# William-wAng618/roboticAttack

Measured on AMD Instinct MI355X. Metric: attack-steps/sec (bs=64, 3x50x50 patch, OpenVLA-7B), higher is better.
Workload: dtype bf16; 1 GPU; UADA_wrapper_ddp inner step: bs=64/rank (global 64), patch 3,50,50, geometry=True, maskidx=[0]; OpenVLA-7B shape, random init; u8 frames resident in HBM; global_batch=64, parallelism=dp1, regions=weak, visible_gpus=1, labelled_rows_per_rank=128, tunableop_entries_loaded_min_over_ranks=173

## Files before the change

include/vaa_model_ops.h:

```cpp
#ifndef VAA_MODEL_OPS_H_
#define VAA_MODEL_OPS_H_
#include <stdint.h>
#ifdef __cplusplus
extern "C" {
#endif
int vaa_model_rope(const uint16_t* x, long sb, long st, long sh, const float* cos_t, const float* sin_t, int B, int T, int H, int hd,
                   float sin_sign, uint16_t* out, void* stream);
int vaa_model_swiglu_fwd(const uint16_t* gate, const uint16_t* up, uint16_t* y, long n, void* stream);
int vaa_model_swiglu_bwd(const uint16_t* dy, const uint16_t* gate, const uint16_t* up, uint16_t* dgate, uint16_t* dup, long n, void* stream);
int vaa_model_scale_add(const uint16_t* x, const uint16_t* a, const uint16_t* ls, uint16_t* out, long rows, int D, void* stream);
int vaa_model_rmsnorm_fwd(const uint16_t* x, const uint16_t* w, uint16_t* h, float* rstd, long rows, int D, float eps, void* stream);
int vaa_model_rmsnorm_bwd(const uint16_t* gh, const uint16_t* gpass, const uint16_t* x, const uint16_t* w, const float* rstd, uint16_t* gx,
                          long rows, int D, void* stream);
int vaa_model_layernorm_fwd(const uint16_t* x, const uint16_t* w, const uint16_t* b, uint16_t* h, float* stats, long rows, int D, float eps,
                            void* stream);
int vaa_model_layernorm_bwd(const uint16_t* gh, const uint16_t* gpass, const uint16_t* x, const uint16_t* w, const float* stats, uint16_t* gx,
                            long rows, int D, void* stream);
int vaa_model_attention_fwd(const uint16_t* q, const int64_t* q_str, const uint16_t* k, const int64_t* k_str, const uint16_t* v,
                            const int64_t* v_str, uint16_t* o, const int64_t* o_str, float* lse, const int32_t* cu_seqlens, int B, int H,
                            int T, int hd, int causal, float scale, void* stream);
int vaa_model_attention_bwd(const uint16_t* q, const int64_t* q_str, const uint16_t* k, const int64_t* k_str, const uint16_t* v,
                            const int64_t* v_str, const uint16_t* o, const int64_t* o_str, const uint16_t* dout, const int64_t* do_str,
                            const float* lse, float* dsum, uint16_t* dq, const int64_t* dq_str, uint16_t* dk, const int64_t* dk_str,
                            uint16_t* dv, const int64_t* dv_str, const float* rope_cos, const float* rope_sin, const int32_t* cu_seqlens, int B,
                            int H, int T, int hd, int causal, float scale, void* stream);
int vaa_model_attention_decode(const uint16_t* q, const int64_t* q_str, const uint16_t* k_new, const int64_t* k_str, const uint16_t* v_new,
                               const int64_t* v_str, uint16_t* kcache, const int64_t* kc_str, uint16_t* vcache, const int64_t* vc_str,
                               const int32_t* pos, const float* cos_t, const float* sin_t, uint16_t* o, const int64_t* o_str, int B, int H,
                               int Tmax, int hd, float scale, void* stream);
int vaa_model_q4_dequant(const uint8_t* codes, const float* absmax, const float* table, int N, int K, uint16_t* out_bf16, void* stream);
int vaa_model_q4_gemv(const uint16_t* x, int M, const uint8_t* codes, const float* absmax, const float* table, int N, int K,
                      const uint16_t* res, uint16_t* y, void* stream);
int vaa_model_q8_act_quant(const uint16_t* x, int M, int K, float threshold, int8_t* xq, float* ascale, int32_t* outliers, void* stream);
int vaa_model_q8_matmul(const int8_t* xq, const float* ascale, const int32_t* outliers, const uint16_t* x, int M, const int8_t* q,
                        const float* wscale, int N, int K, const uint16_t* res, uint16_t* y, int form, void* stream);
#ifdef __cplusplus
}
#endif
#endif
```

roboticattack_amd/_lib.py:

```python
from __future__ import annotations

import ctypes as C
import os

_HERE = os.path.dirname(os.path.abspath(__file__))
LIB_PATH = os.environ.get("VAA_LIB_PATH") or os.path.join(_HERE, "libvaa_hip.so")

VAA_OK = 0
MASK_LT_M20, MASK_NE_M100 = 0, 1
LOSS_UADA, LOSS_UADA_DDP, LOSS_UPA, LOSS_CE = 0, 1, 2, 3
DTYPE_F32, DTYPE_BF16 = 0, 1
LAYOUT_FULL, LAYOUT_ROWS = 0, 1
GRAD_FULL, GRAD_SLICE = 0, 1
SEG_UPA_MAX_GROUPS = 32
OPT_ADAMW_HF, OPT_PGD_SIGN = 0, 1
FRAME_RESIZE_MAX_TAPS = 57

MODEL_OP_EXPORTS = ("vaa_model_rope", "vaa_model_swiglu_fwd", "vaa_model_swiglu_bwd", "vaa_model_rmsnorm_fwd", "vaa_model_rmsnorm_bwd",
                    "vaa_model_attention_fwd", "vaa_model_attention_bwd", "vaa_model_layernorm_fwd", "vaa_model_layernorm_bwd", "vaa_model_scale_add",
                    "vaa_model_attention_decode", "vaa_model_q8_act_quant", "vaa_model_q8_matmul", "vaa_model_q4_dequant", "vaa_model_q4_gemv")

EXPORTS = (
    "vaa_last_error",
    "vaa_version",
    "vaa_device_check",
    "vaa_patch_apply_fwd",
    "vaa_patch_grad_ws_bytes",
    "vaa_patch_grad_gather",
    "vaa_loss_ws_bytes",
    "vaa_loss_fwd_bwd",
    "vaa_loss_fwd_bwd_ex",
    "vaa_patch_update",
    "vaa_patch_apply_eval",
    "vaa_eval_preprocess",
    "vaa_frame_resize_taps_bytes",
    "vaa_frame_resize",
    "vaa_crop_resize_fwd",
    "vaa_crop_resize_bwd",
    "vaa_scene_jitter_ws_bytes",
    "vaa_scene_jitter_fwd",
    "vaa_scene_jitter_bwd",
    "vaa_defocus_blur_fwd",
    "vaa_defocus_blur_bwd",
    "vaa_jpeg_roundtrip_ws_bytes",
    "vaa_jpeg_roundtrip",
    "vaa_patch_embed_grad_ws_bytes",
    "vaa_patch_embed_grad_gather",
    "vaa_patch_embed_packed_elems",
    "vaa_patch_embed_pack_weights",
    "vaa_patch_embed_grad_multi_ws_bytes",
    "vaa_patch_embed_grad_gather_multi",
    "vaa_patch_resize_fwd",
    "vaa_patch_resize_ws_bytes",
    "vaa_patch_resize_bwd",
    "vaa_patch_jitter_fwd",
    "vaa_patch_jitter_ws_bytes",
    "vaa_patch_jitter_bwd",
    "vaa_patch_reg_parts",
    "vaa_patch_reg",
    "vaa_patch_apply_fwd_multi",
    "vaa_patch_grad_gather_multi",
    "vaa_loss_rowmap_bytes",
    "vaa_loss_rowmap_build",
    "vaa_loss_rows_ws_bytes",
    "vaa_loss_rows_fwd_bwd",
    "vaa_patch_apply_fwd_tiles",
    "vaa_patch_grad_partials",
    "vaa_patch_embed_grad_gather_multi_tiles",
    "vaa_patch_embed_grad_gather_tiles",
    "vaa_loss_rows_stats",
    "vaa_head_loss_ws_bytes",
    "vaa_head_loss_rows_applies",
    "vaa_head_loss_rows_stats",
    "vaa_head_loss_rows_finish",
    "vaa_head_slice_applies",
    "vaa_head_slice_ws_bytes",
    "vaa_head_slice_pack",
    "vaa_head_slice_fwd_bwd",
    "vaa_step_epilogue",
    "vaa_step_epilogue_update",
    "vaa_loss_rowmap_seg_bytes",
    "vaa_loss_rowmap_build_seg",
    "vaa_step_epilogue_seg",
    "vaa_step_epilogue_seg_update",
    "vaa_patch_update_seg",
    "vaa_loss_rows_fwd_bwd_seg",
    "vaa_step_epilogue_seg_tail",
    "vaa_step_epilogue_seg_tail_update",
    "vaa_loss_rows_fwd_bwd_seg_upa",
    "vaa_async_error",
    "vaa_prof_start",
    "vaa_prof_stop",
    "vaa_prof_get",
)


class VaaError(RuntimeError):
    pass


_lib = None


# ... 137 lines not shown
    L.vaa_patch_embed_grad_gather_tiles.argtypes = [vp, i32, vp, i32, vp, vp, vp, vp, vp, vp, vp, i32, i32, i32, i32, i32, C.POINTER(f32), i32, vp, vp, sz, vp]
    L.vaa_loss_rows_stats.restype = i32
    L.vaa_loss_rows_stats.argtypes = [vp, i32, vp, i32, i32, i32, i32, i32, C.POINTER(f32), vp, i32, vp, sz, vp]
    L.vaa_head_loss_ws_bytes.restype = sz
    L.vaa_head_loss_ws_bytes.argtypes = [i32, i32]
    L.vaa_head_loss_rows_applies.restype = i32
    L.vaa_head_loss_rows_applies.argtypes = [i32, i32, i32]
    L.vaa_head_loss_rows_stats.restype = i32
    L.vaa_head_loss_rows_stats.argtypes = [vp, vp, i32, vp, i32, i32, i32, i32, i32, C.POINTER(f32), vp, vp, sz, vp, sz, vp, vp]
    L.vaa_head_loss_rows_finish.restype = i32
    L.vaa_head_loss_rows_finish.argtypes = [vp, i32, i32, i32, i32, i32, C.POINTER(f32), vp, sz, vp, sz, vp, vp, vp, vp, vp]
    L.vaa_head_slice_applies.restype = i32
    L.vaa_head_slice_applies.argtypes = [i32, i32, i32]
    L.vaa_head_slice_ws_bytes.restype = sz
    L.vaa_head_slice_ws_bytes.argtypes = [i32]
    L.vaa_head_slice_pack.restype = i32
    L.vaa_head_slice_pack.argtypes = [vp, i32, i32, vp, vp]
    L.vaa_head_slice_fwd_bwd.restype = i32
    L.vaa_head_slice_fwd_bwd.argtypes = [vp, vp, vp, i32, vp, i32, i32, i32, i32, i32, C.POINTER(f32), vp, vp, vp, sz, vp, vp, vp, vp, sz, vp]
    L.vaa_step_epilogue.restype = i32
    L.vaa_step_epilogue.argtypes = [vp, i32, i32, vp, i32, i32, i32, i32, i32, C.POINTER(f32), vp, sz, vp, vp, vp, vp, vp]
    L.vaa_step_epilogue_update.restype = i32
    L.vaa_step_epilogue_update.argtypes = [vp, i32, i32, vp, i32, i32, i32, i32, i32, C.POINTER(f32), vp, sz, vp, vp, vp, vp, vp, vp, vp, i32, f32, f32, f32, f32,
                                           i32, vp, vp]
    L.vaa_loss_rowmap_seg_bytes.restype = sz
    L.vaa_loss_rowmap_seg_bytes.argtypes = [i32, i32, i32]
    L.vaa_loss_rowmap_build_seg.restype = i32
    L.vaa_loss_rowmap_build_seg.argtypes = [vp, i32, i32, i32, vp, sz, vp]
    L.vaa_step_epilogue_seg.restype = i32
    L.vaa_step_epilogue_seg.argtypes = [vp, i32, i32, i32, vp, i32, i32, i32, i32, i32, C.POINTER(f32), vp, sz, vp, vp, vp, vp, vp]
    L.vaa_step_epilogue_seg_update.restype = i32
    L.vaa_step_epilogue_seg_update.argtypes = [vp, i32, i32, i32, vp, i32, i32, i32, i32, i32, C.POINTER(f32), vp, sz, vp, vp, vp, vp, vp, vp, vp, i32, f32,
                                               f32, f32, f32, i32, vp, vp]
    L.vaa_patch_update_seg.restype = i32
    L.vaa_patch_update_seg.argtypes = [vp, vp, vp, vp, i32, i32, i32, f32, f32, f32, f32, i32, f32, f32, vp, vp]
    L.vaa_loss_rows_fwd_bwd_seg.restype = i32
    L.vaa_loss_rows_fwd_bwd_seg.argtypes = [vp, i32, vp, i32, i32, i32, i32, i32, i32, C.POINTER(f32), vp, vp, vp, vp, i32, vp, sz, vp]
    L.vaa_step_epilogue_seg_tail.restype = i32
    L.vaa_step_epilogue_seg_tail.argtypes = [vp, i32, i32, i32, vp, vp, vp]
    L.vaa_step_epilogue_seg_tail_update.restype = i32
    L.vaa_step_epilogue_seg_tail_update.argtypes = [vp, i32, i32, i32, vp, vp, vp, vp, vp, i32, f32, f32, f32, f32, i32, vp, vp]
    L.vaa_loss_rows_fwd_bwd_seg_upa.restype = i32
    L.vaa_loss_rows_fwd_bwd_seg_upa.argtypes = [vp, i32, vp, i32, i32, i32, i32, i32, C.POINTER(f32), vp, vp, vp, vp, vp, sz, vp]
    L.vaa_async_error.restype = i32
    L.vaa_async_error.argtypes = []
    L.vaa_prof_start.restype = i32
    L.vaa_prof_start.argtypes = [i32]
    L.vaa_prof_stop.restype = i32
    L.vaa_prof_stop.argtypes = []
    L.vaa_prof_get.restype = i32
    L.vaa_prof_get.argtypes = [i32, C.POINTER(C.c_char_p), C.POINTER(f32)]
    lng = C.c_long
    L.vaa_model_rope.restype = i32
    L.vaa_model_rope.argtypes = [vp, lng, lng, lng, vp, vp, i32, i32, i32, i32, f32, vp, vp]
    L.vaa_model_swiglu_fwd.restype = i32
    L.vaa_model_swiglu_fwd.argtypes = [vp, vp, vp, lng, vp]
    L.vaa_model_swiglu_bwd.restype = i32
    L.vaa_model_swiglu_bwd.argtypes = [vp, vp, vp, vp, vp, lng, vp]
    L.vaa_model_scale_add.restype = i32
    L.vaa_model_scale_add.argtypes = [vp, vp, vp, vp, lng, i32, vp]
    L.vaa_model_rmsnorm_fwd.restype = i32
    L.vaa_model_rmsnorm_fwd.argtypes = [vp, vp, vp, vp, lng, i32, f32, vp]
    L.vaa_model_rmsnorm_bwd.restype = i32
    L.vaa_model_rmsnorm_bwd.argtypes = [vp, vp, vp, vp, vp, vp, lng, i32, vp]
    L.vaa_model_layernorm_fwd.restype = i32
    L.vaa_model_layernorm_fwd.argtypes = [vp, vp, vp, vp, vp, lng, i32, f32, vp]
    L.vaa_model_layernorm_bwd.restype = i32
    L.vaa_model_layernorm_bwd.argtypes = [vp, vp, vp, vp, vp, vp, lng, i32, vp]
    i64p = C.POINTER(C.c_int64)
    L.vaa_model_attention_fwd.restype = i32
    L.vaa_model_attention_fwd.argtypes = [vp, i64p, vp, i64p, vp, i64p, vp, i64p, vp, vp, i32, i32, i32, i32, i32, f32, vp]
    L.vaa_model_attention_bwd.restype = i32
    L.vaa_model_attention_bwd.argtypes = [vp, i64p, vp, i64p, vp, i64p, vp, i64p, vp, i64p, vp, vp, vp, i64p, vp, i64p, vp, i64p, vp, vp, vp, i32, i32, i32, i32, i32, f32, vp]
    L.vaa_model_attention_decode.restype = i32
    L.vaa_model_attention_decode.argtypes = [vp, i64p, vp, i64p, vp, i64p, vp, i64p, vp, i64p, vp, vp, vp, vp, i64p, i32, i32, i32, i32, f32, vp]
    L.vaa_model_q4_dequant.restype = i32
    L.vaa_model_q4_dequant.argtypes = [vp, vp, C.POINTER(f32), i32, i32, vp, vp]
    L.vaa_model_q4_gemv.restype = i32
    L.vaa_model_q4_gemv.argtypes = [vp, i32, vp, vp, C.POINTER(f32), i32, i32, vp, vp, vp]
    L.vaa_model_q8_act_quant.restype = i32
    L.vaa_model_q8_act_quant.argtypes = [vp, i32, i32, f32, vp, vp, vp, vp]
    L.vaa_model_q8_matmul.restype = i32
    L.vaa_model_q8_matmul.argtypes = [vp, vp, vp, vp, i32, vp, vp, i32, i32, vp, vp, i32, vp]
    _lib = L
    return L


def check(rc: int, what: str) -> None:
    if rc != VAA_OK:
        msg = lib().vaa_last_error().decode("utf-8", "replace")
        raise VaaError(f"{what} failed with code {rc}: {msg}")


def f32x(vals):
    return (C.c_float * len(vals))(*[float(v) for v in vals])
```

roboticattack_amd/model_ops.py:

```python
from __future__ import annotations

import os

import torch

from . import _lib


def enabled(x: torch.Tensor) -> bool:
    return x.is_cuda and x.dtype == torch.bfloat16 and not os.environ.get("VAA_NO_FUSED_MODEL_OPS")


def attention_kernel_enabled(ops_on: bool, hd: int) -> bool:
    return bool(ops_on) and not os.environ.get("VAA_NO_FUSED_ATTENTION") and hd % 8 == 0 and hd <= 128


def attention_enabled(x_bthd: torch.Tensor) -> bool:
    return (attention_kernel_enabled(enabled(x_bthd), x_bthd.shape[-1])
            and all(s % 8 == 0 for s in x_bthd.stride()[:-1]) and x_bthd.stride(-1) == 1)


def _stream():
    return torch.cuda.current_stream().cuda_stream

# ... 55 lines not shown
    @staticmethod
    def forward(ctx, x, a, ls):
        ctx.save_for_backward(ls)
        return _scale_add(x.contiguous(), a.contiguous(), ls.contiguous())

    @staticmethod
    def backward(ctx, g):
        (ls,) = ctx.saved_tensors
        g = g.contiguous()
        da = _scale_add(None, g, ls.contiguous()) if ctx.needs_input_grad[1] else None
        return (g if ctx.needs_input_grad[0] else None), da, None


def scale_add(x: torch.Tensor, a: torch.Tensor, ls: torch.Tensor) -> torch.Tensor:
    if (enabled(x) and a.dtype == x.dtype and ls.dtype == x.dtype and x.shape == a.shape and ls.dim() == 1 and ls.shape[0] == x.shape[-1]
            and x.shape[-1] % 8 == 0 and a.device == x.device and ls.device == x.device and not ls.requires_grad
            and os.environ.get("VAA_MODEL_SCALE_ADD", "1") != "0"):
        return ScaleAddFn.apply(x, a, ls)
    return torch.addcmul(x, a, ls)


class ResidualRMSNormFn(torch.autograd.Function):

    @staticmethod
    def forward(ctx, x, weight, eps):
        x = x.contiguous()
        D = x.shape[-1]
        rows = x.numel() // D
        h = torch.empty_like(x)
        rstd = torch.empty(rows, dtype=torch.float32, device=x.device)
        _lib.check(_lib.lib().vaa_model_rmsnorm_fwd(x.data_ptr(), weight.data_ptr(), h.data_ptr(), rstd.data_ptr(), rows, D, float(eps), _stream()),
                   "vaa_model_rmsnorm_fwd")
        ctx.save_for_backward(x, weight, rstd)
        return x, h

    @staticmethod
    def backward(ctx, g_pass, g_h):
        x, weight, rstd = ctx.saved_tensors
        D = x.shape[-1]
        rows = x.numel() // D
        if g_h is None:
            return g_pass, None, None
        g_h = g_h.contiguous()
        gp = g_pass.contiguous() if g_pass is not None else None
        gx = torch.empty_like(x)
        _lib.check(_lib.lib().vaa_model_rmsnorm_bwd(g_h.data_ptr(), gp.data_ptr() if gp is not None else None, x.data_ptr(), weight.data_ptr(),
                                                    rstd.data_ptr(), gx.data_ptr(), rows, D, _stream()), "vaa_model_rmsnorm_bwd")
        return gx, None, None


class ResidualLayerNormFn(torch.autograd.Function):

    @staticmethod
    def forward(ctx, x, weight, bias, eps):
        x = x.contiguous()
        D = x.shape[-1]
        rows = x.numel() // D
        h = torch.empty_like(x)
        stats = torch.empty((rows, 2), dtype=torch.float32, device=x.device)
        _lib.check(_lib.lib().vaa_model_layernorm_fwd(x.data_ptr(), weight.data_ptr(), bias.data_ptr(), h.data_ptr(), stats.data_ptr(), rows, D,
                                                      float(eps), _stream()), "vaa_model_layernorm_fwd")
        ctx.save_for_backward(x, weight, stats)
        return x, h

    @staticmethod
    def backward(ctx, g_pass, g_h):
        x, weight, stats = ctx.saved_tensors
        D = x.shape[-1]
        rows = x.numel() // D
        if g_h is None:
            return g_pass, None, None, None
        g_h = g_h.contiguous()
        gp = g_pass.contiguous() if g_pass is not None else None
        gx = torch.empty_like(x)
        _lib.check(_lib.lib().vaa_model_layernorm_bwd(g_h.data_ptr(), gp.data_ptr() if gp is not None else None, x.data_ptr(), weight.data_ptr(),
                                                      stats.data_ptr(), gx.data_ptr(), rows, D, _stream()), "vaa_model_layernorm_bwd")
        return gx, None, None, None


def tn_dgrad_enabled() -> bool:
    return not os.environ.get("VAA_NO_TN_DGRAD")


class FrozenLinearsFn(torch.autograd.Function):

    @staticmethod
    def forward(ctx, x, res, *ws):
        x2 = x.reshape(-1, x.shape[-1])
        W, Wt = ws[0::2], ws[1::2]
        ctx.wt = Wt
        ctx.xshape = x.shape
        ctx.has_res = res is not None
        if res is not None:
            return (torch.addmm(res.reshape(-1, W[0].shape[0]), x2, W[0].t()).view(*x.shape[:-1], W[0].shape[0]),)
        return tuple(torch.nn.functional.linear(x2, w).view(*x.shape[:-1], w.shape[0]) for w in W)

    @staticmethod
    def backward(ctx, *dys):
        dx = None
        for dy, wt in zip(dys, ctx.wt):
            if dy is None:
                continue
            d2 = dy.reshape(-1, dy.shape[-1])
            if dx is None:
                dx = torch.nn.functional.linear(d2, wt)
            else:
                dx.addmm_(d2, wt.t())
        dx = dx.view(ctx.xshape) if dx is not None else None
        dres = dys[0] if ctx.has_res else None
        return (dx, dres) + (None,) * (2 * len(ctx.wt))


def _str3(x: torch.Tensor):
    import ctypes

    if x.stride(3) != 1:
        raise ValueError("attention operands need a contiguous head dimension")
    return (ctypes.c_int64 * 3)(x.stride(0), x.stride(1), x.stride(2))


def attention_fwd(q: torch.Tensor, k: torch.Tensor, v: torch.Tensor, causal: bool, scale: float | None = None, cu_seqlens=None, max_len: int = 0):
    Bq, T, H, hd = q.shape
    scale = float(hd) ** -0.5 if scale is None else float(scale)
    o = torch.empty((Bq, T, H, hd), dtype=torch.bfloat16, device=q.device)
    B, Tm = (int(cu_seqlens.numel()) - 1, int(max_len)) if cu_seqlens is not None else (Bq, T)
    lse = torch.empty((B, H, Tm), dtype=torch.float32, device=q.device)
    rc = _lib.lib().vaa_model_attention_fwd(q.data_ptr(), _str3(q), k.data_ptr(), _str3(k), v.data_ptr(), _str3(v), o.data_ptr(), _str3(o),
                                            lse.data_ptr(), cu_seqlens.data_ptr() if cu_seqlens is not None else None, B, H, Tm, hd,
                                            int(bool(causal)), scale, _stream())
    _lib.check(rc, "vaa_model_attention_fwd")
    return o, lse


def attention_bwd(q, k, v, o, lse, dout, causal: bool, scale: float, packed_grad: bool = False, rope=None, cu_seqlens=None, max_len: int = 0):
    Bq, T, H, hd = q.shape
    B, Tm = (int(cu_seqlens.numel()) - 1, int(max_len)) if cu_seqlens is not None else (Bq, T)
    if dout.stride(3) != 1:
        dout = dout.contiguous()
    if packed_grad:
        buf = torch.empty((Bq, T, 3, H, hd), dtype=torch.bfloat16, device=q.device)
        dq, dk, dv = buf[:, :, 0], buf[:, :, 1], buf[:, :, 2]
    else:
        buf = None
        dq, dk, dv = (torch.empty((Bq, T, H, hd), dtype=torch.bfloat16, device=q.device) for _ in range(3))
    dsum = torch.empty((B, H, Tm), dtype=torch.float32, device=q.device)
    rc = _lib.lib().vaa_model_attention_bwd(q.data_ptr(), _str3(q), k.data_ptr(), _str3(k), v.data_ptr(), _str3(v), o.data_ptr(), _str3(o),
                                            dout.data_ptr(), _str3(dout), lse.data_ptr(), dsum.data_ptr(), dq.data_ptr(), _str3(dq),
                                            dk.data_ptr(), _str3(dk), dv.data_ptr(), _str3(dv), rope[0].data_ptr() if rope else None,
                                            rope[1].data_ptr() if rope else None, cu_seqlens.data_ptr() if cu_seqlens is not None else None,
                                            B, H, Tm, hd, int(bool(causal)), float(scale), _stream())
    _lib.check(rc, "vaa_model_attention_bwd")
    return buf if packed_grad else (dq, dk, dv)


def rope_in_attention(hd: int) -> bool:
    return hd in (64, 128)


def _attention_forward(ctx, q, k, v, rope, causal, scale, cu_seqlens, max_len, packed_src):
    scale = float(q.shape[-1]) ** -0.5 if scale is None else float(scale)
    if rope is not None:
        q, k = _rope_launch(q, *rope, 1.0), _rope_launch(k, *rope, 1.0)
    o, lse = attention_fwd(q, k, v, causal, scale, cu_seqlens, max_len)
    operands = (q, k, v) if packed_src is None else (q, k, packed_src) if rope is not None else (packed_src,)
    ctx.save_for_backward(o, lse, *operands, *(rope or ()), *([cu_seqlens] if cu_seqlens is not None else []))
    ctx.attn = (bool(causal), scale, int(max_len), packed_src is not None, rope is not None, cu_seqlens is not None)
    return o


def _attention_backward(ctx, dout):
    causal, scale, max_len, packed, roped, has_cu = ctx.attn
    o, lse, *rest = ctx.saved_tensors
    cu = rest.pop() if has_cu else None
    rope = (rest.pop(-2), rest.pop()) if roped else None
    if packed:
        src = rest.pop()
        rest += [src[:, :, z] for z in range(len(rest), 3)]
    g = attention_bwd(*rest, o, lse, dout, causal, scale, packed_grad=packed, rope=rope, cu_seqlens=cu, max_len=max_len)
    return (*((g,) if packed else g), *(None,) * (2 + (4 if roped else 0)))


class AttentionFn(torch.autograd.Function):

    @staticmethod
    def forward(ctx, q, k, v, causal, scale):
        return _attention_forward(ctx, q, k, v, None, causal, scale, None, 0, None)

    backward = staticmethod(_attention_backward)


class RopeAttentionFn(torch.autograd.Function):

    @staticmethod
# ... 67 lines not shown
```

roboticattack_amd/openvla_model.py:

```python
from __future__ import annotations

import os
import types
from dataclasses import dataclass
from typing import NamedTuple

import torch
import torch.nn as nn
import torch.nn.functional as F

from . import model_ops
from .constants import IGNORE_INDEX, MODEL_VOCAB, N_IMG_TOKENS, PAD_ID


@dataclass
class VitCfg:
    dim: int
    depth: int
    heads: int
    mlp: int
    n_prefix: int
    cls_pos: bool
    layerscale: bool

# ... 84 lines not shown
        self.fc1 = nn.Linear(c.dim, c.mlp)
        self.fc2 = nn.Linear(c.mlp, c.dim)
        self.ls1 = nn.Parameter(torch.ones(c.dim)) if c.layerscale else None
        self.ls2 = nn.Parameter(torch.ones(c.dim)) if c.layerscale else None

    def forward(self, x):
        B, T, D = x.shape
        fused_ln = _fused(model_ops.enabled(x), D)
        x, h = _norm(self.norm1, x, fused_ln)
        qkv = self.qkv(h).view(B, T, 3, self.heads, D // self.heads)
        if model_ops.attention_enabled(qkv):
            a = model_ops.PackedAttentionFn.apply(qkv, False, None).reshape(B, T, D)
        else:
            qkv = qkv.permute(2, 0, 3, 1, 4)
            a = F.scaled_dot_product_attention(qkv[0], qkv[1], qkv[2]).transpose(1, 2).reshape(B, T, D)
        a = self.proj(a)
        x = model_ops.scale_add(x, a, self.ls1) if self.ls1 is not None else x + a
        x, h = _norm(self.norm2, x, fused_ln)
        h = self.fc2(F.gelu(self.fc1(h)))
        return model_ops.scale_add(x, h, self.ls2) if self.ls2 is not None else x + h


class Vit(nn.Module):

    def __init__(self, c: VitCfg):
        super().__init__()
        self.c = c
        self.patch_embed = nn.Conv2d(3, c.dim, kernel_size=14, stride=14)
        self.pos_embed = nn.Parameter(torch.zeros(1, N_IMG_TOKENS + (1 if c.cls_pos else 0), c.dim))
        self.prefix = nn.Parameter(torch.zeros(1, c.n_prefix, c.dim)) if c.n_prefix else None
        self.blocks = nn.ModuleList([VitBlock(c) for _ in range(c.depth - 1)])

    def embed_params(self):
        from . import ops
        w = self.patch_embed.weight
        if not (w.is_cuda and w.dtype == torch.bfloat16 and self.c.dim % 64 == 0):
            return w.detach().reshape(self.c.dim, 588), self.patch_embed.bias.detach(), None
        hit = getattr(self, "_embed_wp", None)
        if hit is None or hit[0] != w._version or hit[1] is not w:
            hit = (w._version, w, ops.pack_embed_weights(w.detach().reshape(self.c.dim, 588).t().contiguous()))
            self._embed_wp = hit
        return w.detach().reshape(self.c.dim, 588), self.patch_embed.bias.detach(), hit[2]

    def forward(self, img, embedded=None):
        if embedded is not None:
            x = embedded
        else:
            B0 = img.shape[0]
            tiles = img.reshape(B0, 3, 16, 14, 16, 14).permute(0, 2, 4, 1, 3, 5).reshape(B0, 256, 588)
            x = F.linear(tiles, self.patch_embed.weight.reshape(self.c.dim, 588), self.patch_embed.bias)
        if self.prefix is not None and self.c.cls_pos:
            B = x.shape[0]
            cls = self.prefix[:, :1].expand(B, -1, -1)
            reg = self.prefix[:, 1:].expand(B, -1, -1)
            x = torch.cat([cls, x], dim=1) + self.pos_embed
            x = torch.cat([x[:, :1], reg, x[:, 1:]], dim=1)
        elif self.prefix is not None:
            x = torch.cat([self.prefix.expand(x.shape[0], -1, -1), x + self.pos_embed], dim=1)
        else:
            x = x + self.pos_embed
        for blk in self.blocks:
            x = blk(x)
        return x[:, self.c.n_prefix :]


class RMSNorm(nn.Module):
    def __init__(self, dim, eps):
        super().__init__()
        self.weight = nn.Parameter(torch.ones(dim))
        self.eps = eps

    def forward(self, x):
        return F.rms_norm(x, (x.shape[-1],), self.weight, self.eps)


def _rope(q, k, cos, sin):
    def rot(x):
        x1, x2 = x[..., : x.shape[-1] // 2], x[..., x.shape[-1] // 2 :]
        return torch.cat((-x2, x1), dim=-1)

    return q * cos + rot(q) * sin, k * cos + rot(k) * sin


class Bf16Projections:

    def __init__(self, layer):
        self.layer = layer

    def qkv(self, h2, fused, gemv):
        L = self.layer
        if fused:
            return F.linear(h2, L._wcat(("q_proj", "k_proj", "v_proj"))[0])
        return torch.stack([L.q_proj(h2), L.k_proj(h2), L.v_proj(h2)], dim=1).view(h2.shape[0], -1)

    def o(self, a2, res, gemv):
        return torch.addmm(res, a2, self.layer.o_proj.weight.t())

    def gate_up(self, h2, fused, gemv):
        return self.layer.gate_proj(h2), self.layer.up_proj(h2)

    def down(self, y2, res, fused_mlp, gemv):
        if fused_mlp:
            return torch.addmm(res, y2, self.layer.down_proj.weight.t())
        return res + self.layer.down_proj(y2)


class LlamaLayer(nn.Module):
    quant_type = None

    def __init__(self, c: OpenVLACfg):
        super().__init__()
        d = c.llm_dim
        self.heads = c.llm_heads
        self.input_layernorm = RMSNorm(d, c.rms_eps)
        self.q_proj = nn.Linear(d, d, bias=False)
        self.k_proj = nn.Linear(d, d, bias=False)
        self.v_proj = nn.Linear(d, d, bias=False)
        self.o_proj = nn.Linear(d, d, bias=False)
        self.post_attention_layernorm = RMSNorm(d, c.rms_eps)
        self.gate_proj = nn.Linear(d, c.llm_mlp, bias=False)
        self.up_proj = nn.Linear(d, c.llm_mlp, bias=False)
        self.down_proj = nn.Linear(c.llm_mlp, d, bias=False)
        self._wt_cache = {}
        self.projections = Bf16Projections(self)

    def _wt(self, name):
        w = getattr(self, name).weight
        hit = self._wt_cache.get(name)
        if hit is None or hit[0] != w._version or hit[1] is not w:
            hit = (w._version, w, w.detach().t().contiguous())
            self._wt_cache[name] = hit
        return hit[2]

    def _wcat(self, names):
        ws = [getattr(self, n).weight for n in names]
        key = "+".join(names)
        ver = tuple(w._version for w in ws)
        hit = self._wt_cache.get(key)
        if hit is None or hit[0] != ver or any(a is not b for a, b in zip(hit[1], ws)):
            w = torch.cat([w.detach() for w in ws], 0).contiguous()
            hit = (ver, ws, w, w.t().contiguous())
            self._wt_cache[key] = hit
        return hit[2], hit[3]

    def _lin(self, x, names, res=None):
        ws = [w for n in names for w in (getattr(self, n).weight, self._wt(n))]
        return model_ops.FrozenLinearsFn.apply(x, res, *ws)

    def _qkv(self, h, r):
        B, T, _ = h.shape
        if r.qkv_cat:
            (qkv,) = model_ops.FrozenLinearsFn.apply(h, None, *self._wcat(("q_proj", "k_proj", "v_proj")))
            return qkv.view(B, T, 3, self.heads, -1)
        qkv = self._lin(h, ("q_proj", "k_proj", "v_proj")) if r.tn else (self.q_proj(h), self.k_proj(h), self.v_proj(h))
        return tuple(t.view(B, T, self.heads, -1) for t in qkv)

    def _attention(self, qkv, r, cos, sin, rope_tab):
        if r.attention == "rope_packed":
            return model_ops.RopePackedAttentionFn.apply(qkv, *rope_tab, True, None, r.cu, r.max_len)
        q, k, v = qkv if isinstance(qkv, tuple) else (qkv[:, :, z] for z in range(3))
        if r.attention == "rope":
            return model_ops.RopeAttentionFn.apply(q, k, v, *rope_tab, True, None, r.cu, r.max_len)
        if r.attention != "stock_sdpa":
            q, k = model_ops.RopeFn.apply(q, *rope_tab), model_ops.RopeFn.apply(k, *rope_tab)
        if r.attention == "rope_fn_attention":
            return model_ops.AttentionFn.apply(q, k, v, True, None)
        q, k, v = q.transpose(1, 2), k.transpose(1, 2), v.transpose(1, 2)
        if r.attention == "stock_sdpa":
            q, k = _rope(q, k, cos, sin)
        return F.scaled_dot_product_attention(q, k, v, is_causal=True).transpose(1, 2)

    def _proj_res(self, name, a, x, r):
        if r.tn:
            return self._lin(a, (name,), res=x)[0]
        return torch.addmm(x.reshape(-1, x.shape[-1]), a.reshape(-1, a.shape[-1]), getattr(self, name).weight.t()).view(x.shape)

    def _mlp(self, x, h, r):
        if not (r.fused and (h.shape[0] * h.shape[1] * self.gate_proj.out_features) % 8 == 0):
            return x + self.down_proj(F.silu(self.gate_proj(h)) * self.up_proj(h))
        g, u = self._lin(h, ("gate_proj", "up_proj")) if r.tn else (self.gate_proj(h), self.up_proj(h))
        return self._proj_res("down_proj", model_ops.SwiGLUFn.apply(g, u), x, r)

    def forward(self, x, cos, sin, rope_tab=None, rows=None, pack=None, route=None):
        if self.quant_type:
            from . import quant

            quant.refuse_training("LlamaLayer.forward", self.quant_type)
        B, T, D = x.shape
        r = route if route is not None else _route(rows=B * T, pack=pack, **_facts(x, self.heads, rope_tab))
        x, h = _norm(self.input_layernorm, x, r.fused)
        a = self._attention(self._qkv(h, r), r, cos, sin, rope_tab).reshape(B, T, D)
        if rows is not None:
            a, x = (t.reshape(-1, D).index_select(0, rows)[None] for t in (a, x))
        x = self._proj_res("o_proj", a, x, r)
        x, h = _norm(self.post_attention_layernorm, x, r.fused)
        x = self._mlp(x, h, r)
        return x[0] if rows is not None else x

    def _infer_fused(self, x) -> bool:
        return _fused(model_ops.enabled(x), x.shape[-1], x.shape[-1] // self.heads)

    def _infer_norm_qkv(self, x, fused, gemv):
        B, T, D = x.shape
        h = _norm(self.input_layernorm, x, fused)[1].reshape(-1, D)
        return self.projections.qkv(h, fused, gemv).view(B, T, 3, self.heads, D // self.heads)

    def _infer_o_mlp(self, x, a, fused, gemv):
        B, T, D = x.shape
        proj = self.projections
        x2 = proj.o(a.reshape(-1, D), x.reshape(-1, D), gemv)
        h = _norm(self.post_attention_layernorm, x2.view(B, T, D), fused)[1].reshape(-1, D)
        g, u = proj.gate_up(h, fused, gemv)
        fused_mlp = fused and (B * T * g.shape[1]) % 8 == 0
        y = model_ops.SwiGLUFn.apply(g, u) if fused_mlp else F.silu(g) * u
        return proj.down(y, x2, fused_mlp, gemv).view(B, T, D)

    @torch.no_grad()
    def prefill(self, x, rope_tab, cache):
        B, T, D = x.shape
        fused = self._infer_fused(x)
        qkv = self._infer_norm_qkv(x, fused, gemv=False)
        cos, sin = rope_tab[0][:T], rope_tab[1][:T]
        if fused:
            q, k = model_ops.RopeFn.apply(qkv[:, :, 0], cos, sin), model_ops.RopeFn.apply(qkv[:, :, 1], cos, sin)
        else:
            c, s = (torch.cat([t, t], -1).to(x.dtype)[None, :, None, :] for t in (cos, sin))
            q, k = _rope(qkv[:, :, 0], qkv[:, :, 1], c, s)
        v = qkv[:, :, 2]
        if fused and model_ops.attention_enabled(q):
            a = model_ops.attention_fwd(q, k, v, True)[0]
        else:
            a = F.scaled_dot_product_attention(q.transpose(1, 2), k.transpose(1, 2), v.transpose(1, 2), is_causal=True).transpose(1, 2)
        cache[0][:, :T] = k
        cache[1][:, :T] = v
        return self._infer_o_mlp(x, a.reshape(B, T, D), fused, gemv=False)

    @torch.no_grad()
    def decode_step(self, x, pos, rope_tab, cache):
        B, _, D = x.shape
        fused = self._infer_fused(x)
        qkv = self._infer_norm_qkv(x, fused, gemv=True)[:, 0]
        a = model_ops.attention_decode(qkv[:, 0], qkv[:, 1], qkv[:, 2], cache[0], cache[1], pos, rope_tab[0], rope_tab[1])
        return self._infer_o_mlp(x, a.reshape(B, 1, D), fused, gemv=True)


class SeqPack:

    def __init__(self, attention_mask: torch.Tensor):
        B, L = attention_mask.shape
        self.T_pad = N_IMG_TOKENS + L
        lens = (attention_mask.sum(1).to(torch.int64) + N_IMG_TOKENS).tolist()
        dev = attention_mask.device
        cu = [0]
        for n in lens:
            cu.append(cu[-1] + int(n))
        self.total = cu[-1]
        fill = (-cu[-1]) % 256
        if fill:
# ... 289 lines not shown
```

Before: 2.217 attack-steps/s.

## Route residual linear projections through native hipBLASLt GEMM with TunableOp selections

Adds a native hipBLASLt/rocBLAS GEMM entry point with per-thread cached plans, a registered per-stream workspace, and algorithm selection read from the PyTorch TunableOp CSV. The residual-add projections (o_proj, down_proj) now call it, with C=residual and beta=1, in place of torch.addmm, and a new autograd function covers the untied frozen-weight path. The aim is to skip PyTorch's addmm dispatch and copy overhead and to reuse tuned solutions directly. It adds per-call ctypes overhead and a new code path that may pick different kernels. Weight cache keys now also include the data pointer and shape.

```diff
diff --git a/include/vaa_model_ops.h b/include/vaa_model_ops.h
--- a/include/vaa_model_ops.h
+++ b/include/vaa_model_ops.h
@@ -1,5 +1,6 @@
 #ifndef VAA_MODEL_OPS_H_
 #define VAA_MODEL_OPS_H_
+#include <stddef.h>
 #include <stdint.h>
 #ifdef __cplusplus
 extern "C" {
@@ -34,6 +35,10 @@
 int vaa_model_q8_act_quant(const uint16_t* x, int M, int K, float threshold, int8_t* xq, float* ascale, int32_t* outliers, void* stream);
 int vaa_model_q8_matmul(const int8_t* xq, const float* ascale, const int32_t* outliers, const uint16_t* x, int M, const int8_t* q,
                         const float* wscale, int N, int K, const uint16_t* res, uint16_t* y, int form, void* stream);
+int vaa_model_gemm(const uint16_t* A, long lda, const uint16_t* W, long ldw, const uint16_t* bias, const uint16_t* C, long ldc, uint16_t* D, long ldd,
+                   long M, long N, long K, void* stream);
+int vaa_model_gemm_workspace(void* ws, size_t ws_bytes, void* stream);
+int vaa_model_gemm_tuning_file(const char* path, int device);
 #ifdef __cplusplus
 }
 #endif
diff --git a/roboticattack_amd/_lib.py b/roboticattack_amd/_lib.py
--- a/roboticattack_amd/_lib.py
+++ b/roboticattack_amd/_lib.py
@@ -18,7 +18,8 @@
 
 MODEL_OP_EXPORTS = ("vaa_model_rope", "vaa_model_swiglu_fwd", "vaa_model_swiglu_bwd", "vaa_model_rmsnorm_fwd", "vaa_model_rmsnorm_bwd",
                     "vaa_model_attention_fwd", "vaa_model_attention_bwd", "vaa_model_layernorm_fwd", "vaa_model_layernorm_bwd", "vaa_model_scale_add",
-                    "vaa_model_attention_decode", "vaa_model_q8_act_quant", "vaa_model_q8_matmul", "vaa_model_q4_dequant", "vaa_model_q4_gemv")
+                    "vaa_model_attention_decode", "vaa_model_gemm", "vaa_model_gemm_workspace", "vaa_model_gemm_tuning_file",
+                    "vaa_model_q8_act_quant", "vaa_model_q8_matmul", "vaa_model_q4_dequant", "vaa_model_q4_gemv")
 
 EXPORTS = (
     "vaa_last_error",
@@ -322,6 +323,12 @@
     L.vaa_model_q8_act_quant.argtypes = [vp, i32, i32, f32, vp, vp, vp, vp]
     L.vaa_model_q8_matmul.restype = i32
     L.vaa_model_q8_matmul.argtypes = [vp, vp, vp, vp, i32, vp, vp, i32, i32, vp, vp, i32, vp]
+    L.vaa_model_gemm.restype = i32
+    L.vaa_model_gemm.argtypes = [vp, lng, vp, lng, vp, vp, lng, vp, lng, lng, lng, lng, vp]
+    L.vaa_model_gemm_workspace.restype = i32
+    L.vaa_model_gemm_workspace.argtypes = [vp, sz, vp]
+    L.vaa_model_gemm_tuning_file.restype = i32
+    L.vaa_model_gemm_tuning_file.argtypes = [C.c_char_p, i32]
     _lib = L
     return L
 
diff --git a/roboticattack_amd/csrc/vaa_gemm.hip b/roboticattack_amd/csrc/vaa_gemm.hip
--- /dev/null
+++ b/roboticattack_amd/csrc/vaa_gemm.hip
@@ -0,0 +1,352 @@
+#include <hipblaslt/hipblaslt-ext.hpp>
+#include <hipblaslt/hipblaslt.h>
+#include <rocblas/rocblas.h>
+
+#include <mutex>
+#include <vector>
+
+#include "../../include/vaa_model_ops.h"
+#include "vaa_common.h"
+#include "vaa_gemm_csv.h"
+
+namespace {
+
+using vaa::set_error;
+namespace csv = vaa::gemm_csv;
+
+constexpr int kMaxDevices = 64;
+
+struct WsEntry {
+    int dev;
+    void* stream;
+    void* ptr;
+    size_t bytes;
+};
+std::mutex g_mu;
+csv::Table* g_table[kMaxDevices] = {};
+unsigned g_table_gen = 0;
+std::vector<WsEntry> g_ws;
+
+bool workspace_of(int dev, void* stream, void** ptr, size_t* bytes) {
+    std::lock_guard<std::mutex> lk(g_mu);
+    for (const WsEntry& e : g_ws)
+        if (e.dev == dev && e.stream == stream) {
+            *ptr = e.ptr;
+            *bytes = e.bytes;
+            return true;
+        }
+    *ptr = nullptr;
+    *bytes = 0;
+    return false;
+}
+
+struct Key {
+    int dev;
+    long M, N, K, lda, ldw, ldc, ldd;
+    bool bias, has_c;
+    bool operator==(const Key& o) const {
+        return dev == o.dev && M == o.M && N == o.N && K == o.K && lda == o.lda && ldw == o.ldw && ldc == o.ldc && ldd == o.ldd && bias == o.bias &&
+               has_c == o.has_c;
+    }
+};
+
+struct Plan {
+    Key key;
+    int backend;
+    hipblasLtMatmulDesc_t desc;
+    hipblasLtMatrixLayout_t la, lb, lc, ld;
+    hipblasLtMatmulAlgo_t algo;
+    size_t ws_need;
+    int solution;
+    bool rb_checked;
+    const void* bias_set;
+};
+
+struct ThreadState {
+    hipblasLtHandle_t lt[kMaxDevices];
+    rocblas_handle rb[kMaxDevices];
+    std::vector<Plan>* plans;
+    unsigned gen;
+};
+thread_local ThreadState t_state = {};
+
+const char* lt_status(hipblasStatus_t s) {
+    switch (s) {
+        case HIPBLAS_STATUS_SUCCESS: return "success";
+        case HIPBLAS_STATUS_NOT_INITIALIZED: return "not initialized";
+        case HIPBLAS_STATUS_ALLOC_FAILED: return "allocation failed";
+        case HIPBLAS_STATUS_INVALID_VALUE: return "invalid value";
+        case HIPBLAS_STATUS_NOT_SUPPORTED: return "not supported";
+        case HIPBLAS_STATUS_EXECUTION_FAILED: return "execution failed";
+        default: return "error";
+    }
+}
+
+void destroy_plan(Plan& p) {
+    if (p.la) hipblasLtMatrixLayoutDestroy(p.la);
+    if (p.lb) hipblasLtMatrixLayoutDestroy(p.lb);
+    if (p.lc) hipblasLtMatrixLayoutDestroy(p.lc);
+    if (p.ld) hipblasLtMatrixLayoutDestroy(p.ld);
+    if (p.desc) hipblasLtMatmulDescDestroy(p.desc);
+    p.la = p.lb = p.lc = p.ld = nullptr;
+    p.desc = nullptr;
+}
+
+int heuristic(hipblasLtHandle_t h, Plan& p, size_t ws_bytes) {
+    hipblasLtMatmulPreference_t pref = nullptr;
+    hipblasStatus_t s = hipblasLtMatmulPreferenceCreate(&pref);
+    if (s == HIPBLAS_STATUS_SUCCESS) {
+        uint64_t w = ws_bytes;
+        s = hipblasLtMatmulPreferenceSetAttribute(pref, HIPBLASLT_MATMUL_PREF_MAX_WORKSPACE_BYTES, &w, sizeof(w));
+    }
+    hipblasLtMatmulHeuristicResult_t res[1];
+    int n = 0;
+    if (s == HIPBLAS_STATUS_SUCCESS) s = hipblasLtMatmulAlgoGetHeuristic(h, p.desc, p.la, p.lb, p.lc, p.ld, pref, 1, res, &n);
+    if (pref) hipblasLtMatmulPreferenceDestroy(pref);
+    if (s != HIPBLAS_STATUS_SUCCESS || n < 1) {
+        set_error("vaa_model_gemm: hipBLASLt has no algorithm for M=%ld N=%ld K=%ld (%s)", p.key.M, p.key.N, p.key.K, lt_status(s));
+        return VAA_E_UNSUPPORTED;
+    }
+    p.backend = csv::kHipblaslt;
+    p.algo = res[0].algo;
+    p.ws_need = res[0].workspaceSize;
+    return VAA_OK;
+}
+
+void say_fallback(const Key& k, const char* sel, int index, const char* why) {
+    fprintf(stderr, "vaa_model_gemm: tuned selection %s_%d rejected for tn_%ld_%ld_%ld (%s); using the hipBLASLt heuristic\n", sel, index, k.N, k.M,
+            k.K, why);
+}
+
+int rocblas_call(rocblas_handle h, const Plan& p, const void* A, const void* W, const void* C, void* D, hipStream_t st, uint32_t flags) {
+    const float alpha = 1.0f, beta = p.key.has_c ? 1.0f : 0.0f;
+    rocblas_status s = rocblas_set_stream(h, st);
+    if (s != rocblas_status_success) return (int)s;
+    const Key& k = p.key;
+    return (int)rocblas_gemm_ex(h, rocblas_operation_transpose, rocblas_operation_none, (rocblas_int)k.N, (rocblas_int)k.M, (rocblas_int)k.K, &alpha, W,
+                                rocblas_datatype_bf16_r, (rocblas_int)k.ldw, A, rocblas_datatype_bf16_r, (rocblas_int)k.lda, &beta, C ? C : D,
+                                rocblas_datatype_bf16_r, (rocblas_int)(C ? k.ldc : k.ldd), D, rocblas_datatype_bf16_r, (rocblas_int)k.ldd,
+                                rocblas_datatype_f32_r, rocblas_gemm_algo_solution_index, p.solution, flags);
+}
+
+int build_plan(const Key& key, size_t ws_bytes, Plan* out) {
+    ThreadState& ts = t_state;
+    Plan p = {};
+    p.key = key;
+    hipblasLtHandle_t h = ts.lt[key.dev];
+    hipblasStatus_t s = hipblasLtMatmulDescCreate(&p.desc, HIPBLAS_COMPUTE_32F, HIP_R_32F);
+    const hipblasOperation_t opT = HIPBLAS_OP_T, opN = HIPBLAS_OP_N;
+    if (s == HIPBLAS_STATUS_SUCCESS) s = hipblasLtMatmulDescSetAttribute(p.desc, HIPBLASLT_MATMUL_DESC_TRANSA, &opT, sizeof(opT));
+    if (s == HIPBLAS_STATUS_SUCCESS) s = hipblasLtMatmulDescSetAttribute(p.desc, HIPBLASLT_MATMUL_DESC_TRANSB, &opN, sizeof(opN));
+    if (s == HIPBLAS_STATUS_SUCCESS && key.bias) {
+        const hipblasLtEpilogue_t ep = HIPBLASLT_EPILOGUE_BIAS;
+        const hipDataType bt = HIP_R_16BF;
+        s = hipblasLtMatmulDescSetAttribute(p.desc, HIPBLASLT_MATMUL_DESC_EPILOGUE, &ep, sizeof(ep));
+        if (s == HIPBLAS_STATUS_SUCCESS) s = hipblasLtMatmulDescSetAttribute(p.desc, HIPBLASLT_MATMUL_DESC_BIAS_DATA_TYPE, &bt, sizeof(bt));
+    }
+    if (s == HIPBLAS_STATUS_SUCCESS) s = hipblasLtMatrixLayoutCreate(&p.la, HIP_R_16BF, key.K, key.N, key.ldw);
+    if (s == HIPBLAS_STATUS_SUCCESS) s = hipblasLtMatrixLayoutCreate(&p.lb, HIP_R_16BF, key.K, key.M, key.lda);
+    if (s == HIPBLAS_STATUS_SUCCESS) s = hipblasLtMatrixLayoutCreate(&p.lc, HIP_R_16BF, key.N, key.M, key.has_c ? key.ldc : key.ldd);
+    if (s == HIPBLAS_STATUS_SUCCESS) s = hipblasLtMatrixLayoutCreate(&p.ld, HIP_R_16BF, key.N, key.M, key.ldd);
+    if (s != HIPBLAS_STATUS_SUCCESS) {
+        set_error("vaa_model_gemm: hipBLASLt descriptor setup failed (%s)", lt_status(s));
+        destroy_plan(p);
+        return VAA_E_LAUNCH;
+    }
+    const csv::Row* row = nullptr;
+    {
+        std::lock_guard<std::mutex> lk(g_mu);
+        if (g_table[key.dev]) row = csv::find(*g_table[key.dev], key.bias, key.N, key.M, key.K);
+    }
+    bool chosen = false;
+    if (row && row->backend == csv::kHipblaslt) {
+        std::vector<int> idx(1, row->index);
+        std::vector<hipblasLtMatmulHeuristicResult_t> res;
+        const float alpha = 1.0f, beta = key.has_c ? 1.0f : 0.0f;
+        size_t need = 0;
+        const char* why = nullptr;
+        if (hipblaslt_ext::getAlgosFromIndex(h, idx, res) != HIPBLAS_STATUS_SUCCESS || res.empty()) why = "unknown index";
+        else if (hipblaslt_ext::matmulIsAlgoSupported(h, p.desc, &alpha, p.la, p.lb, &beta, p.lc, p.ld, res[0].algo, need) != HIPBLAS_STATUS_SUCCESS)
+            why = "not supported for these arguments";
+        else if (need > ws_bytes) why = "needs more workspace than registered";
+        if (!why) {
+            p.backend = csv::kHipblaslt;
+            p.algo = res[0].algo;
+            p.ws_need = need;
+            chosen = true;
+        } else {
+            say_fallback(key, "Gemm_Hipblaslt", row->index, why);
+        }
+    } else if (row && row->backend == csv::kRocblas) {
+        const long lim = 0x7fffffffL;
+        p.backend = csv::kRocblas;
+        p.solution = row->index;
+        const char* why = nullptr;
+        if (key.bias) why = "rocBLAS has no bias epilogue";
+        else if (key.M > lim || key.N > lim || key.K > lim || key.lda > lim || key.ldw > lim || key.ldc > lim || key.ldd > lim) why = "32-bit sizes";
+        else {
+            if (!ts.rb[key.dev] && rocblas_create_handle(&ts.rb[key.dev]) != rocblas_status_success) {
+                ts.rb[key.dev] = nullptr;
+                why = "no rocBLAS handle";
+            }
+        }
+        if (!why) chosen = true;
+        else say_fallback(key, "Gemm_Rocblas", row->index, why);
+    }
+    if (!chosen) {
+        const int rc = heuristic(h, p, ws_bytes);
+        if (rc != VAA_OK) {
+            destroy_plan(p);
+            return rc;
+        }
+    }
+    *out = p;
+    return VAA_OK;
+}
+
+}
+
+extern "C" {
+
+int vaa_model_gemm_tuning_file(const char* path, int device) {
+    if (device < 0 || device >= kMaxDevices) {
+        set_error("vaa_model_gemm_tuning_file: bad device %d", device);
+        return VAA_E_INVALID;
+    }
+    csv::Table* t = nullptr;
+    if (path && path[0]) {
+        t = new csv::Table();
+        if (!csv::load(path, t)) {
+            delete t;
+            set_error("vaa_model_gemm_tuning_file: cannot open %s", path);
+            return VAA_E_INVALID;
+        }
+    }
+    std::lock_guard<std::mutex> lk(g_mu);
+    g_table[device] = t;
+    ++g_table_gen;
+    return VAA_OK;
+}
+
+int vaa_model_gemm_workspace(void* ws, size_t ws_bytes, void* stream) {
+    int dev = 0;
+    if (hipGetDevice(&dev) != hipSuccess || dev < 0 || dev >= kMaxDevices) {
+        set_error("vaa_model_gemm_workspace: no current device");
+        return VAA_E_NODEVICE;
+    }
+    if ((ws == nullptr) != (ws_bytes == 0) || ((uintptr_t)ws & 255u)) {
+        set_error("vaa_model_gemm_workspace: the workspace must be 256-byte aligned, and NULL exactly when its size is 0");
+        return VAA_E_INVALID;
+    }
+    std::lock_guard<std::mutex> lk(g_mu);
+    for (WsEntry& e : g_ws)
+        if (e.dev == dev && e.stream == stream) {
+            e.ptr = ws;
+            e.bytes = ws_bytes;
+            return VAA_OK;
+        }
+    g_ws.push_back(WsEntry{dev, stream, ws, ws_bytes});
+    return VAA_OK;
+}
+
+int vaa_model_gemm(const uint16_t* A, long lda, const uint16_t* W, long ldw, const uint16_t* bias, const uint16_t* C, long ldc, uint16_t* D, long ldd,
+                   long M, long N, long K, void* stream) {
+    const char* who = "vaa_model_gemm";
+    if (M < 0 || N < 1 || K < 1) {
+        set_error("%s: bad sizes (M=%ld N=%ld K=%ld)", who, M, N, K);
+        return VAA_E_INVALID;
+    }
+    if (M == 0) return VAA_OK;
+    if (!A || !W || !D) {
+        set_error("%s: null pointer argument", who);
+        return VAA_E_INVALID;
+    }
+    if (lda < K || ldw < K || ldd < N || (C && ldc < N)) {
+        set_error("%s: a leading dimension is smaller than its row (lda=%ld ldw=%ld ldc=%ld ldd=%ld for N=%ld K=%ld)", who, lda, ldw, ldc, ldd, N, K);
+        return VAA_E_INVALID;
+    }
+    if (C && C != D) {
+        const uintptr_t c0 = (uintptr_t)C, c1 = c0 + ((size_t)(M - 1) * ldc + N) * 2, d0 = (uintptr_t)D, d1 = d0 + ((size_t)(M - 1) * ldd + N) * 2;
+        if (c0 < d1 && d0 < c1) {
+            set_error("%s: C and D overlap without being the same matrix", who);
+            return VAA_E_INVALID;
+        }
+    }
+    int dev = 0;
+    if (hipGetDevice(&dev) != hipSuccess || dev < 0 || dev >= kMaxDevices) {
+        set_error("%s: no current device", who);
+        return VAA_E_NODEVICE;
+    }
+    ThreadState& ts = t_state;
+    if (!ts.plans) ts.plans = new std::vector<Plan>();
+    {
+        unsigned gen;
+        {
+            std::lock_guard<std::mutex> lk(g_mu);
+            gen = g_table_gen;
+        }
+        if (gen != ts.gen) {
+            for (Plan& p : *ts.plans) destroy_plan(p);
+            ts.plans->clear();
+            ts.gen = gen;
+        }
+    }
+    if (!ts.lt[dev]) {
+        const hipblasStatus_t s = hipblasLtCreate(&ts.lt[dev]);
+        if (s != HIPBLAS_STATUS_SUCCESS) {
+            ts.lt[dev] = nullptr;
+            set_error("%s: hipblasLtCreate failed (%s)", who, lt_status(s));
+            return VAA_E_LAUNCH;
+        }
+    }
+    void* ws = nullptr;
+    size_t ws_bytes = 0;
+    workspace_of(dev, stream, &ws, &ws_bytes);
+    const Key key = {dev, M, N, K, lda, ldw, C ? ldc : 0, ldd, bias != nullptr, C != nullptr};
+    Plan* p = nullptr;
+    for (Plan& q : *ts.plans)
+        if (q.key == key) {
+            p = &q;
+            break;
+        }
+    if (!p) {
+        Plan fresh;
+        const int rc = build_plan(key, ws_bytes, &fresh);
+        if (rc != VAA_OK) return rc;
+        ts.plans->push_back(fresh);
+        p = &ts.plans->back();
+    }
+    const hipStream_t st = (hipStream_t)stream;
+    if (p->backend == csv::kRocblas) {
+        int s = p->rb_checked ? (int)rocblas_status_success : rocblas_call(ts.rb[dev], *p, A, W, C, D, st, rocblas_gemm_flags_check_solution_index);
+        p->rb_checked = true;
+        if (s == (int)rocblas_status_success) s = rocblas_call(ts.rb[dev], *p, A, W, C, D, st, rocblas_gemm_flags_none);
+        if (s == (int)rocblas_status_success) return vaa::check_launch(who);
+        say_fallback(key, "Gemm_Rocblas", p->solution, rocblas_status_to_string((rocblas_status)s));
+        const int rc = heuristic(ts.lt[dev], *p, ws_bytes);
+        if (rc != VAA_OK) return rc;
+    }
+    if (p->ws_need > ws_bytes) {
+        set_error("%s: workspace %zu B < required %zu B (vaa_model_gemm_workspace registers one per stream)", who, ws_bytes, p->ws_need);
+        return VAA_E_WORKSPACE;
+    }
+    if (key.bias && p->bias_set != bias) {
+        const void* b = bias;
+        const hipblasStatus_t s = hipblasLtMatmulDescSetAttribute(p->desc, HIPBLASLT_MATMUL_DESC_BIAS_POINTER, &b, sizeof(b));
+        if (s != HIPBLAS_STATUS_SUCCESS) {
+            set_error("%s: setting the bias pointer failed (%s)", who, lt_status(s));
+            return VAA_E_LAUNCH;
+        }
+        p->bias_set = bias;
+    }
+    const float alpha = 1.0f, beta = C ? 1.0f : 0.0f;
+    const hipblasStatus_t s = hipblasLtMatmul(ts.lt[dev], p->desc, &alpha, W, p->la, A, p->lb, &beta, C ? (const void*)C : (const void*)D, p->lc, D, p->ld,
+                                              &p->algo, ws, ws_bytes, st);
+    if (s != HIPBLAS_STATUS_SUCCESS) {
+        set_error("%s: hipblasLtMatmul failed (%s) for M=%ld N=%ld K=%ld", who, lt_status(s), M, N, K);
+        return VAA_E_LAUNCH;
+    }
+    return vaa::check_launch(who);
+}
+
+}
diff --git a/roboticattack_amd/csrc/vaa_gemm_csv.h b/roboticattack_amd/csrc/vaa_gemm_csv.h
--- /dev/null
+++ b/roboticattack_amd/csrc/vaa_gemm_csv.h
@@ -0,0 +1,120 @@
+#pragma once
+
+#include <stdio.h>
+#include <string.h>
+
+#include <string>
+#include <vector>
+
+namespace vaa {
+namespace gemm_csv {
+
+enum Backend { kDefault = 0, kHipblaslt = 1, kRocblas = 2 };
+
+struct Row {
+    bool bias;
+    long N, M, K;
+    int backend;
+    int index;
+};
+
+struct Table {
+    std::vector<Row> rows;
+    int validators = 0;
+    int skipped = 0;
+};
+
+inline long parse_pos(const char* s, const char* e, long limit) {
+    if (s >= e || e - s > 18) return -1;
+    long v = 0;
+    for (const char* p = s; p < e; ++p) {
+        if (*p < '0' || *p > '9') return -1;
+        v = v * 10 + (*p - '0');
+    }
+    return (v >= 1 && v <= limit) ? v : -1;
+}
+
+inline int parse_line(const char* s, size_t len, Row* out) {
+    const char* e = s + len;
+    const char* f[4];
+    const char* fe[4];
+    int nf = 0;
+    const char* p = s;
+    while (nf < 4) {
+        f[nf] = p;
+        while (p < e && *p != ',') ++p;
+        fe[nf] = p;
+        ++nf;
+        if (p == e) break;
+        ++p;
+    }
+    auto is = [&](int i, const char* lit) { return (size_t)(fe[i] - f[i]) == strlen(lit) && memcmp(f[i], lit, strlen(lit)) == 0; };
+    auto starts = [&](int i, const char* lit) { return (size_t)(fe[i] - f[i]) >= strlen(lit) && memcmp(f[i], lit, strlen(lit)) == 0; };
+    if (nf >= 3 && is(0, "Validator")) return 2;
+    if (nf < 3) return 0;
+    Row r;
+    if (is(0, "GemmTunableOp_BFloat16_TN")) r.bias = false;
+    else if (is(0, "GemmAndBiasTunableOp_BFloat16_TN")) r.bias = true;
+    else return 0;
+    if (!starts(1, "tn_")) return 0;
+    const char* q = f[1] + 3;
+    long v[3];
+    for (int i = 0; i < 3; ++i) {
+        const char* u = q;
+        while (u < fe[1] && *u != '_') ++u;
+        if (u == fe[1]) return 0;
+        v[i] = parse_pos(q, u, 1L << 40);
+        if (v[i] < 0) return 0;
+        q = u + 1;
+    }
+    if (fe[1] - q < 3 || memcmp(q, "ld_", 3) != 0) return 0;
+    r.N = v[0]; r.M = v[1]; r.K = v[2];
+    if (is(2, "Default")) {
+        r.backend = kDefault;
+        r.index = 0;
+    } else {
+        const char* lit = nullptr;
+        if (starts(2, "Gemm_Hipblaslt_")) r.backend = kHipblaslt, lit = "Gemm_Hipblaslt_";
+        else if (starts(2, "Gemm_Rocblas_")) r.backend = kRocblas, lit = "Gemm_Rocblas_";
+        else return 0;
+        const long idx = parse_pos(f[2] + strlen(lit), fe[2], 0x7fffffffL);
+        if (idx < 0) return 0;
+        r.index = (int)idx;
+    }
+    *out = r;
+    return 1;
+}
+
+inline bool load(const char* path, Table* t) {
+    *t = Table();
+    FILE* fp = path ? fopen(path, "rb") : nullptr;
+    if (!fp) return false;
+    std::string line;
+    bool more = true;
+    while (more) {
+        line.clear();
+        int c;
+        while ((c = fgetc(fp)) != EOF && c != '\n') {
+            if (line.size() < 4096) line.push_back((char)c);
+        }
+        more = c != EOF;
+        while (!line.empty() && (line.back() == '\r' || line.back() == ' ')) line.pop_back();
+        if (line.empty()) continue;
+        Row r;
+        const int kind = parse_line(line.data(), line.size(), &r);
+        if (kind == 1) t->rows.push_back(r);
+        else if (kind == 2) ++t->validators;
+        else ++t->skipped;
+    }
+    fclose(fp);
+    return true;
+}
+
+inline const Row* find(const Table& t, bool bias, long N, long M, long K) {
+    for (const Row& r : t.rows)
+        if (r.bias == bias && r.N == N && r.M == M && r.K == K) return &r;
+    return nullptr;
+}
+
+}
+}
diff --git a/roboticattack_amd/model_ops.py b/roboticattack_amd/model_ops.py
--- a/roboticattack_amd/model_ops.py
+++ b/roboticattack_amd/model_ops.py
@@ -161,6 +161,79 @@
     return not os.environ.get("VAA_NO_TN_DGRAD")
 
 
+def native_gemm_enabled() -> bool:
+    return os.environ.get("VAA_NATIVE_GEMM", "1") != "0"
+
+
+def native_gemm_applies(a: torch.Tensor, w: torch.Tensor, res=None) -> bool:
+    return (native_gemm_enabled() and enabled(a) and w.dtype == a.dtype and w.device == a.device and w.dim() == 2
+            and (res is None or (res.dtype == a.dtype and res.device == a.device)))
+
+
+GEMM_WS_BYTES = 64 << 20
+_gemm_streams = set()
+_gemm_devices = set()
+
+
+def _tunableop_file():
+    try:
+        import torch.cuda.tunable as tunable
+
+        if not tunable.is_enabled():
+            return None
+        path = tunable.get_filename()
+        if not path or not os.path.exists(path):
+            return None
+        with open(path) as f:
+            want = {tuple(line.strip().split(",")[1:3]) for line in f if line.startswith("Validator,")}
+        have = {tuple(str(v) for v in kv) for kv in tunable.get_validators()}
+        return path if want <= have else None
+    except Exception:
+        return None
+
+
+def _gemm_setup(dev: torch.device, stream: int) -> None:
+    L = _lib.lib()
+    idx = dev.index if dev.index is not None else torch.cuda.current_device()
+    if idx not in _gemm_devices:
+        path = _tunableop_file()
+        _lib.check(L.vaa_model_gemm_tuning_file(path.encode() if path else None, idx), "vaa_model_gemm_tuning_file")
+        _gemm_devices.add(idx)
+    if (idx, stream) not in _gemm_streams:
+        from . import ops
+
+        ws = ops._workspace(dev, GEMM_WS_BYTES, "gemm")
+        _lib.check(L.vaa_model_gemm_workspace(ws.data_ptr(), ws.numel(), stream), "vaa_model_gemm_workspace")
+        _gemm_streams.add((idx, stream))
+
+
+def _rows(t: torch.Tensor, width: int) -> torch.Tensor:
+    return t if t.stride(1) == 1 and (t.shape[0] == 1 or t.stride(0) >= width) else t.contiguous()
+
+
+def gemm(a2: torch.Tensor, w: torch.Tensor, bias=None, res=None) -> torch.Tensor:
+    M, K = a2.shape
+    N = w.shape[0]
+    a2, w = _rows(a2, K), _rows(w, K)
+    res = _rows(res, N) if res is not None else None
+    bias = bias.contiguous() if bias is not None else None
+    out =torch.empty((M, N), dtype=a2.dtype, device=a2.device)
+    with torch.cuda.device(a2.device):
+        st = _stream()
+        _gemm_setup(a2.device, st)
+        rc = _lib.lib().vaa_model_gemm(a2.data_ptr(), max(a2.stride(0), K), w.data_ptr(), max(w.stride(0), K),
+                                       bias.contiguous().data_ptr() if bias is not None else None, res.data_ptr() if res is not None else None,
+                                       max(res.stride(0), N) if res is not None else 0, out.data_ptr(), N, M, N, K, st)
+    _lib.check(rc, "vaa_model_gemm")
+    return out
+
+
+def linear_res(a2: torch.Tensor, w: torch.Tensor, res: torch.Tensor) -> torch.Tensor:
+    if native_gemm_applies(a2, w, res):
+        return gemm(a2, w, None, res)
+    return torch.addmm(res, a2, w.t())
+
+
 class FrozenLinearsFn(torch.autograd.Function):
 
     @staticmethod
@@ -171,7 +244,7 @@
         ctx.xshape = x.shape
         ctx.has_res = res is not None
         if res is not None:
-            return (torch.addmm(res.reshape(-1, W[0].shape[0]), x2, W[0].t()).view(*x.shape[:-1], W[0].shape[0]),)
+            return (linear_res(x2, W[0], res.reshape(-1, W[0].shape[0])).view(*x.shape[:-1], W[0].shape[0]),)
         return tuple(torch.nn.functional.linear(x2, w).view(*x.shape[:-1], w.shape[0]) for w in W)
 
     @staticmethod
@@ -188,6 +261,21 @@
         dx = dx.view(ctx.xshape) if dx is not None else None
         dres = dys[0] if ctx.has_res else None
         return (dx, dres) + (None,) * (2 * len(ctx.wt))
+
+
+class ResidualLinearFn(torch.autograd.Function):
+
+    @staticmethod
+    def forward(ctx, a, res, w):
+        ctx.save_for_backward(w)
+        ctx.ashape = a.shape
+        return linear_res(a.reshape(-1, a.shape[-1]), w, res.reshape(-1, w.shape[0])).view(res.shape)
+
+    @staticmethod
+    def backward(ctx, dy):
+        (w,) = ctx.saved_tensors
+        da = (dy.reshape(-1, dy.shape[-1]) @ w).view(ctx.ashape) if ctx.needs_input_grad[0] else None
+        return da, (dy if ctx.needs_input_grad[1] else None), None
 
 
 def _str3(x: torch.Tensor):
diff --git a/roboticattack_amd/openvla_model.py b/roboticattack_amd/openvla_model.py
--- a/roboticattack_amd/openvla_model.py
+++ b/roboticattack_amd/openvla_model.py
@@ -190,6 +190,10 @@
     return q * cos + rot(q) * sin, k * cos + rot(k) * sin
 
 
+def _wkey(w):
+    return (w._version, w.data_ptr(), tuple(w.shape))
+
+
 class Bf16Projections:
 
     def __init__(self, layer):
@@ -202,14 +206,14 @@
         return torch.stack([L.q_proj(h2), L.k_proj(h2), L.v_proj(h2)], dim=1).view(h2.shape[0], -1)
 
     def o(self, a2, res, gemv):
-        return torch.addmm(res, a2, self.layer.o_proj.weight.t())
+        return model_ops.linear_res(a2, self.layer.o_proj.weight, res)
 
     def gate_up(self, h2, fused, gemv):
         return self.layer.gate_proj(h2), self.layer.up_proj(h2)
 
     def down(self, y2, res, fused_mlp, gemv):
         if fused_mlp:
-            return torch.addmm(res, y2, self.layer.down_proj.weight.t())
+            return model_ops.linear_res(y2, self.layer.down_proj.weight, res)
         return res + self.layer.down_proj(y2)
 
 
@@ -235,15 +239,15 @@
     def _wt(self, name):
         w = getattr(self, name).weight
         hit = self._wt_cache.get(name)
-        if hit is None or hit[0] != w._version or hit[1] is not w:
-            hit = (w._version, w, w.detach().t().contiguous())
+        if hit is None or hit[0] != _wkey(w) or hit[1] is not w:
+            hit = (_wkey(w), w, w.detach().t().contiguous())
             self._wt_cache[name] = hit
         return hit[2]
 
     def _wcat(self, names):
         ws = [getattr(self, n).weight for n in names]
         key = "+".join(names)
-        ver = tuple(w._version for w in ws)
+        ver = tuple(_wkey(w) for w in ws)
         hit = self._wt_cache.get(key)
         if hit is None or hit[0] != ver or any(a is not b for a, b in zip(hit[1], ws)):
             w = torch.cat([w.detach() for w in ws], 0).contiguous()
@@ -281,7 +285,10 @@
     def _proj_res(self, name, a, x, r):
         if r.tn:
             return self._lin(a, (name,), res=x)[0]
-        return torch.addmm(x.reshape(-1, x.shape[-1]), a.reshape(-1, a.shape[-1]), getattr(self, name).weight.t()).view(x.shape)
+        w = getattr(self, name).weight
+        if not w.requires_grad and model_ops.native_gemm_applies(a, w, x):
+            return model_ops.ResidualLinearFn.apply(a, x, w)
+        return torch.addmm(x.reshape(-1, x.shape[-1]), a.reshape(-1, a.shape[-1]), w.t()).view(x.shape)
 
     def _mlp(self, x, h, r):
         if not (r.fused and (h.shape[0] * h.shape[1] * self.gate_proj.out_features) % 8 == 0):
```

Result: no change. 2.233 attack-steps/s, median of 6 (+0.8%).
